# vfrantc/Bayesian-Enhancement-Model

Hardware: AMD Instinct MI355X
Metric: images/sec (whole node) CG_UNet N=8 Bayesian eval @256x256 (higher is better)
Workload: dtype f32

## Files before the change

bayesian-enhancement-model_amd/csrc/chan_attn.hip:

```cpp
#include "bem_common.h"

namespace {

constexpr int ATT_C = 32;
constexpr int ATT_CHUNK = 2048;
__global__ __launch_bounds__(256) void attn_stats_kernel(const float* __restrict__ f1, const float* __restrict__ f2,
                                                         double* __restrict__ stats, int L) {
    __shared__ double t1[ATT_C][65], t2[ATT_C][65];
    const int b = blockIdx.y;
    const int p0 = blockIdx.x * ATT_CHUNK;
    const int i0 = (threadIdx.x >> 4) * 2, j0 = (threadIdx.x & 15) * 2;
    double a00 = 0, a01 = 0, a10 = 0, a11 = 0, r0 = 0, r1 = 0, c0 = 0, c1 = 0;
    const float* F1 = f1 + (int64_t)b * ATT_C * L;
    const float* F2 = f2 + (int64_t)b * ATT_C * L;
    const int pend = min(p0 + ATT_CHUNK, L);
    for (int ps = p0; ps < pend; ps += 64) {
        __syncthreads();
        for (int i = threadIdx.x; i < ATT_C * 64; i += 256) {
            const int c = i >> 6, pp = i & 63;
            const int p = ps + pp;
            t1[c][pp] = p < pend ? (double)F1[(int64_t)c * L + p] : 0.0;
            t2[c][pp] = p < pend ? (double)F2[(int64_t)c * L + p] : 0.0;
        }
        __syncthreads();
#pragma unroll 8
        for (int pp = 0; pp < 64; ++pp) {
            const double u0 = t1[i0][pp], u1 = t1[i0 + 1][pp], v0 = t2[j0][pp], v1 = t2[j0 + 1][pp];
            a00 = fma(u0, v0, a00); a01 = fma(u0, v1, a01); a10 = fma(u1, v0, a10); a11 = fma(u1, v1, a11);
            if (j0 == 0) { r0 += u0; r1 += u1; }
            if (i0 == 0) { c0 += v0; c1 += v1; }
        }
    }
    double* S = stats + (int64_t)b * (ATT_C * ATT_C + 2 * ATT_C);
    atomicAdd(&S[i0 * ATT_C + j0], a00);
    atomicAdd(&S[i0 * ATT_C + j0 + 1], a01);
    atomicAdd(&S[(i0 + 1) * ATT_C + j0], a10);
    atomicAdd(&S[(i0 + 1) * ATT_C + j0 + 1], a11);
    if (j0 == 0) { atomicAdd(&S[ATT_C * ATT_C + i0], r0); atomicAdd(&S[ATT_C * ATT_C + i0 + 1], r1); }
    if (i0 == 0) { atomicAdd(&S[ATT_C * ATT_C + ATT_C + j0], c0); atomicAdd(&S[ATT_C * ATT_C + ATT_C + j0 + 1], c1); }
}

__device__ __forceinline__ double mm(const double (*A)[33], const double (*Bm)[33], int i, int j) {
    double s = 0;
#pragma unroll 8
    for (int k = 0; k < ATT_C; ++k) s = fma(A[i][k], Bm[k][j], s);
    return s;
}

__global__ __launch_bounds__(1024) void attn_fold_kernel(const double* __restrict__ stats, const float* __restrict__ aw,
                                                         const float* __restrict__ fw, const float* __restrict__ fb,
                                                         float* __restrict__ Wp, float* __restrict__ bias_out, int L) {
    __shared__ double X[ATT_C][33], Y[ATT_C][33], Z[ATT_C][33], M1[ATT_C][33], M2[ATT_C][33];
    __shared__ double va[ATT_C], vb[ATT_C], c1[ATT_C], c2[ATT_C], rowred[ATT_C];
    const int i = threadIdx.x >> 5, j = threadIdx.x & 31;
    const int b = blockIdx.x;
    const double* S = stats + (int64_t)b * (ATT_C * ATT_C + 2 * ATT_C);
    const double* s1 = S + ATT_C * ATT_C;
    const double* s2 = s1 + ATT_C;
    constexpr int WSZ = ATT_C * ATT_C + ATT_C;
    auto Wm = [&](int m, int r, int c) -> double { return (double)aw[m * WSZ + r * ATT_C + c]; };
    auto Bv = [&](int m, int r) -> double { return (double)aw[m * WSZ + ATT_C * ATT_C + r]; };
    const double scale = 1.0 / sqrt((double)ATT_C);
    for (int br = 0; br < 2; ++br) {
        const int mq = br ? 3 : 0, mk = br ? 4 : 1, mv = br ? 5 : 2, mo = br ? 7 : 6;
        const double* sq = br ? s2 : s1;
        const double* sk = br ? s1 : s2;
        __syncthreads();
        X[i][j] = br ? S[j * ATT_C + i] : S[i * ATT_C + j];
        Y[i][j] = Wm(mk, j, i);
        Z[i][j] = Wm(mq, i, j);
        if (i == 0) {
            double u = 0, t = 0;
            for (int k = 0; k < ATT_C; ++k) { u += Wm(mq, j, k) * sq[k]; t += Wm(mk, j, k) * sk[k]; }
            va[j] = u;
            vb[j] = t;
        }
        __syncthreads();
        const double t1 = mm(Z, X, i, j);
        __syncthreads();
        Z[i][j] = t1;
        __syncthreads();
        double g = mm(Z, Y, i, j);
        g += va[i] * Bv(mk, j) + Bv(mq, i) * vb[j] + (double)L * Bv(mq, i) * Bv(mk, j);
        g *= scale;
        __syncthreads();
        X[i][j] = g;
        __syncthreads();
        if (j == 0) {
            double m = X[i][0];
            for (int k = 1; k < ATT_C; ++k) m = fmax(m, X[i][k]);
            rowred[i] = m;
        }
        __syncthreads();
        const double e = exp(g - rowred[i]);
        __syncthreads();
        X[i][j] = e;
        __syncthreads();
        if (j == 0) {
            double s = 0;
            for (int k = 0; k < ATT_C; ++k) s += X[i][k];
            rowred[i] = s;
        }
        __syncthreads();
        const double pr = e / rowred[i];
        __syncthreads();
        X[i][j] = pr;
        Y[i][j] = Wm(mv, i, j);
        Z[i][j] = Wm(mo, i, j);
        __syncthreads();
        const double pv = mm(X, Y, i, j);
        if (j == 0) {
            double s = 0;
            for (int k = 0; k < ATT_C; ++k) s += X[i][k] * Bv(mv, k);
            va[i] = s;
        }
        __syncthreads();
        Y[i][j] = pv;
        __syncthreads();
        const double mres = mm(Z, Y, i, j);
        if (j == 0) {
            double s = Bv(mo, i);
            for (int k = 0; k < ATT_C; ++k) s += Z[i][k] * va[k];
            (br ? c2 : c1)[i] = s;
        }
        (br ? M2 : M1)[i][j] = mres;
    }
    __syncthreads();
    X[i][j] = (double)fw[i * 64 + j];
    Y[i][j] = (double)fw[i * 64 + 32 + j];
    __syncthreads();
    const double left = X[i][j] + mm(Y, M2, i, j);
    const double right = mm(X, M1, i, j) + Y[i][j];
    float* wp = Wp + (int64_t)b * (32 * 64);
    wp[i * 64 + j] = (float)left;
    wp[i * 64 + 32 + j] = (float)right;
    if (j == 0) {
        double s = (double)fb[i];
        for (int k = 0; k < ATT_C; ++k) s += X[i][k] * c1[k] + Y[i][k] * c2[k];
        bias_out[(int64_t)b * 32 + i] = (float)s;
    }
}

}

extern "C" int bem_attn_stats_f64(const float* f1, const float* f2, double* stats, int B, int L, void* stream) {
    BEM_REQUIRE(f1 && f2 && stats, "attn_stats: null tensor");
    BEM_REQUIRE(B >= 0 && B <= 65535 && L > 0, "attn_stats: bad shape");
    if (B == 0) return BEM_OK;
    hipStream_t s = (hipStream_t)stream;
    BEM_ZERO(stats, sizeof(double) * (size_t)B * (ATT_C * ATT_C + 2 * ATT_C), s, "attn_stats");
    dim3 grid(cdiv(L, ATT_CHUNK), B);
    attn_stats_kernel<<<grid, 256, 0, s>>>(f1, f2, stats, L);
    return bem_check_launch("attn_stats");
}

extern "C" int bem_attn_fold_f32(const double* stats, const float* attn_w, const float* fuse_w, const float* fuse_b,
                                 float* Wp_out, float* bias_out, int B, int L, void* stream) {
    BEM_REQUIRE(stats && attn_w && fuse_w && fuse_b && Wp_out && bias_out, "attn_fold: null tensor");
    BEM_REQUIRE(B >= 0 && L > 0, "attn_fold: bad shape");
    if (B == 0) return BEM_OK;
    attn_fold_kernel<<<B, 1024, 0, (hipStream_t)stream>>>(stats, attn_w, fuse_w, fuse_b, Wp_out, bias_out, L);
    return bem_check_launch("attn_fold");
}
```

bayesian-enhancement-model_amd/csrc/pack.hip:

```cpp
#include "bem_common.h"
#include "x6_common.h"

namespace {

__global__ void pack_pw_weight_kernel(const float* __restrict__ W, float* __restrict__ Wp, int M, int K, int MT, int KS) {
    const int64_t per = (int64_t)MT * KS * 64;
    const int64_t i = (int64_t)blockIdx.x * blockDim.x + threadIdx.x;
    if (i >= per) return;
    const int lane = (int)(i & 63);
    const int64_t t = i >> 6;
    const int st = (int)(t % KS), mt = (int)(t / KS);
    const int row = mt * 32 + (lane & 31), col = 2 * st + (lane >> 5);
    const int set = blockIdx.y;
    Wp[(int64_t)set * per + i] = (row < M && col < K) ? W[((int64_t)set * M + row) * K + col] : 0.f;
}

__device__ __forceinline__ void pack_x6_item(int64_t i, const float* __restrict__ W, u32x4* __restrict__ Wp, int M, int K, int MT, int KB,
                                             int64_t ss, int64_t rs, int64_t cs) {
    const int lane = (int)(i & 63);
    const int64_t blk = i >> 6;
    const int kb = (int)(blk % KB), mt = (int)((blk / KB) % MT);
    const int64_t set = blk / ((int64_t)KB * MT);
    const int row = mt * 32 + (lane & 31), k0 = kb * 16 + (lane >> 5) * 8;
    float v[8];
#pragma unroll
    for (int e = 0; e < 8; ++e) v[e] = (row < M && k0 + e < K) ? W[set * ss + row * rs + (k0 + e) * cs] : 0.f;
    u32x4 h, m, l;
    split8(v, h, m, l);
    u32x4* o = Wp + ((set * MT + mt) * KB + kb) * 3 * 64 + lane;
    o[0] = h; o[64] = m; o[128] = l;
}

__global__ void pack_x6_kernel(const float* __restrict__ W, u32x4* __restrict__ Wp, int M, int K, int MT, int KB, int64_t total,
                               int64_t ss, int64_t rs, int64_t cs) {
    const int64_t i = bem_gid1d();
    if (i >= total) return;
    pack_x6_item(i, W, Wp, M, K, MT, KB, ss, rs, cs);
}

struct packjob { const float* src; int64_t out; int32_t M, K; int64_t rs, cs, items, pad0, pad1; };
static_assert(sizeof(packjob) == 8 * 8, "packjob is eight 64-bit words (bem.modules.BayesBank builds it as an int64 table)");

__global__ __launch_bounds__(256) void pack_x6_jobs_kernel(const packjob* __restrict__ jobs, const int32_t* __restrict__ blks, float* __restrict__ arena) {
    const packjob jb = jobs[blks[2 * blockIdx.x]];
    const int64_t i = (int64_t)blks[2 * blockIdx.x + 1] * 256 + threadIdx.x;
    if (i >= jb.items) return;
    pack_x6_item(i, jb.src, reinterpret_cast<u32x4*>(arena + jb.out), jb.M, jb.K, (jb.M + 31) / 32, (jb.K + 15) / 16, 0, jb.rs, jb.cs);
}

__device__ __forceinline__ void sample_pack_x6_item(int64_t i, const float* __restrict__ mu, const float* __restrict__ rho,
                                                    const float* __restrict__ eps_in, u32x4* __restrict__ Wp, int M, int K, int MT, int KB,
                                                    uint64_t seed, uint64_t stream_id, int sigma_given) {
    const int lane = (int)(i & 63);
    const int64_t blk = i >> 6;
    const int kb = (int)(blk % KB), mt = (int)((blk / KB) % MT);
    const int64_t set = blk / ((int64_t)KB * MT);
    const int row = mt * 32 + (lane & 31), k0 = kb * 16 + (lane >> 5) * 8;
    float v[8];
    const int64_t g0 = set * M * K + (int64_t)row * K + k0;
    float z[3][4];
    if (!eps_in && row < M) {
#pragma unroll
        for (int q = 0; q < 3; ++q) philox_normal4((g0 >> 2) + q, seed, stream_id, z[q]);
    }
#pragma unroll
    for (int e = 0; e < 8; ++e) {
        v[e] = 0.f;
        if (row < M && k0 + e < K) {
            const int64_t idx = (int64_t)row * K + k0 + e, gi = g0 + e;
            const int off = (int)(g0 & 3);
            const float zsel = off == 0 ? z[e >> 2][e & 3] : off == 1 ? z[(e + 1) >> 2][(e + 1) & 3]
                             : off == 2 ? z[(e + 2) >> 2][(e + 2) & 3] : z[(e + 3) >> 2][(e + 3) & 3];
            const float eps = eps_in ? eps_in[gi] : zsel;
            v[e] = mu[idx] + (sigma_given ? rho[idx] : log1pf(expf(rho[idx]))) * eps;
        }
    }
    u32x4 h, m, l;
    split8(v, h, m, l);
    u32x4* o = Wp + ((set * MT + mt) * KB + kb) * 3 * 64 + lane;
    o[0] = h; o[64] = m; o[128] = l;
}

__global__ void sample_pack_x6_kernel(const float* __restrict__ mu, const float* __restrict__ rho, const float* __restrict__ eps_in,
                                      u32x4* __restrict__ Wp, int M, int K, int MT, int KB, int64_t total, uint64_t seed, uint64_t stream_id,
                                      const uint64_t* __restrict__ stream_add, int sigma_given) {
    const int64_t i = bem_gid1d();
    if (i >= total) return;
    if (stream_add) stream_id += stream_add[0];
    sample_pack_x6_item(i, mu, rho, eps_in, Wp, M, K, MT, KB, seed, stream_id, sigma_given);
}

__global__ void randn_kernel(float* __restrict__ out, int64_t total, uint64_t seed, uint64_t stream_id, const uint64_t* __restrict__ stream_add) {
    const int64_t i = bem_gid1d();
    if (stream_add) stream_id += stream_add[0];
    if (i < total) out[i] = philox_normal(i, seed, stream_id);
}

__global__ void bnn_sample_kernel(const float* __restrict__ mu, const float* __restrict__ rho,
                                  const float* __restrict__ eps_in, float* __restrict__ out, int64_t n, int64_t total,
                                  uint64_t seed, uint64_t stream_id, const uint64_t* __restrict__ stream_add) {
    const int64_t j = bem_gid1d();
    const int64_t i0 = 4 * j;
    if (i0 >= total) return;
    if (stream_add) stream_id += stream_add[0];
    float z[4] = {0.f, 0.f, 0.f, 0.f};
    if (!eps_in) philox_normal4(j, seed, stream_id, z);
#pragma unroll
    for (int q = 0; q < 4; ++q) {
        const int64_t i = i0 + q;
        if (i < total) {
            const int64_t e = i % n;
            const float eps = eps_in ? eps_in[i] : z[q];
            out[i] = mu[e] + log1pf(expf(rho[e])) * eps;
        }
    }
}

struct ebank_seg { const float* mu; const float* sig; int64_t out; int64_t n; int32_t M, K; uint64_t counter; int64_t items; int64_t total; };
static_assert(sizeof(ebank_seg) == 8 * 8, "ebank_seg is eight 64-bit words (bem.modules.EvalSampleBank builds it as an int64 table)");
struct ebank_blk { int32_t seg; int32_t first; };

__global__ __launch_bounds__(256) void ebank_sample_kernel(const ebank_seg* __restrict__ segs, const ebank_blk* __restrict__ blks,
                                                           float* __restrict__ arena, uint64_t seed, uint64_t stream_base) {
    const ebank_blk bk = blks[blockIdx.x];
    const ebank_seg sg = segs[bk.seg];
    const int64_t i = (int64_t)bk.first * 256 + threadIdx.x;
    if (i >= sg.items) return;
    const uint64_t sid = stream_base + sg.counter;
    float* out = arena + sg.out;
    if (sg.K > 0) {
        sample_pack_x6_item(i, sg.mu, sg.sig, nullptr, reinterpret_cast<u32x4*>(out), sg.M, sg.K, (sg.M + 31) / 32, (sg.K + 15) / 16, seed, sid, 1);
        return;
    }
    const int64_t i0 = 4 * i, total = sg.total;
    float z[4];
    philox_normal4(i, seed, sid, z);
#pragma unroll
    for (int q = 0; q < 4; ++q) {
        const int64_t e = i0 + q;
        if (e < total) {
            const int64_t k = e % sg.n;
            out[e] = sg.mu[k] + log1pf(expf(sg.sig[k])) * z[q];
        }
    }
}

}

extern "C" int64_t bem_pw_packed_elems(int M, int K) { return (int64_t)cdiv(M, 32) * cdiv(K, 2) * 64; }

extern "C" int bem_pack_pw_weight_f32(const float* W, float* Wp, int nsets, int M, int K, void* stream) {
    BEM_REQUIRE(W && Wp, "pack_pw_weight: null tensor");
    BEM_REQUIRE(nsets >= 0 && nsets <= 65535 && M > 0 && K > 0, "pack_pw_weight: bad shape");
    if (nsets == 0) return BEM_OK;
    const int MT = cdiv(M, 32), KS = cdiv(K, 2);
    dim3 grid((unsigned)cdiv64((int64_t)MT * KS * 64, 256), nsets);
    pack_pw_weight_kernel<<<grid, 256, 0, (hipStream_t)stream>>>(W, Wp, M, K, MT, KS);
    return bem_check_launch("pack_pw_weight");
}

extern "C" int bem_bnn_sample_f32(const float* mu, const float* rho, const float* eps_in, float* out, int nsets,
                                  int64_t n, uint64_t seed, uint64_t stream_id, const uint64_t* stream_add, void* stream) {
    BEM_REQUIRE(mu && rho && out, "bnn_sample: null tensor");
    BEM_REQUIRE(nsets >= 0 && n >= 0, "bnn_sample: bad shape");
    const int64_t total = (int64_t)nsets * n;
    if (total == 0) return BEM_OK;
    bnn_sample_kernel<<<GRID1D(cdiv64(total, 4)), 256, 0, (hipStream_t)stream>>>(mu, rho, eps_in, out, n, total, seed, stream_id, stream_add);
    return bem_check_launch("bnn_sample");
}

extern "C" int bem_randn_f32(float* out, int64_t n, uint64_t seed, uint64_t stream_id, const uint64_t* stream_add, void* stream) {
    BEM_REQUIRE(out && n >= 0, "randn: bad arguments");
    if (n == 0) return BEM_OK;
    randn_kernel<<<GRID1D(n), 256, 0, (hipStream_t)stream>>>(out, n, seed, stream_id, stream_add);
    return bem_check_launch("randn");
}

extern "C" int bem_bnn_ebank_sample_f32(const void* segs, const void* blks, int nblk, float* arena, uint64_t seed, uint64_t stream_base,
                                        void* stream) {
    BEM_REQUIRE(segs && blks && arena && nblk > 0, "bnn_ebank_sample: bad arguments");
    BEM_REQUIRE(((uintptr_t)arena & 15) == 0, "bnn_ebank_sample: the arena must be 16-byte aligned");
    ebank_sample_kernel<<<nblk, 256, 0, (hipStream_t)stream>>>((const ebank_seg*)segs, (const ebank_blk*)blks, arena, seed, stream_base);
    return bem_check_launch("bnn_ebank_sample");
}

extern "C" int bem_bnn_sample_pack_x6(const float* mu, const float* rho, const float* eps_in, float* Wp, int nsets, int M, int K,
                                      uint64_t seed, uint64_t stream_id, const uint64_t* stream_add, int sigma_given, void* stream) {
    BEM_REQUIRE(mu && rho && Wp, "bnn_sample_pack_x6: null tensor");
    BEM_REQUIRE(nsets >= 0 && M > 0 && K > 0, "bnn_sample_pack_x6: bad shape");
    BEM_REQUIRE(((uintptr_t)Wp & 15) == 0, "bnn_sample_pack_x6: output must be 16-byte aligned");
    if (nsets == 0) return BEM_OK;
    const int MT = cdiv(M, 32), KB = cdiv(K, 16);
    const int64_t total = (int64_t)nsets * MT * KB * 64;
    sample_pack_x6_kernel<<<GRID1D(total), 256, 0, (hipStream_t)stream>>>(mu, rho, eps_in, reinterpret_cast<u32x4*>(Wp), M, K, MT, KB,
                                                                                       total, seed, stream_id, stream_add, sigma_given);
    return bem_check_launch("bnn_sample_pack_x6");
}

extern "C" int64_t bem_pw_x6_packed_elems(int M, int K) {
    return (int64_t)cdiv(M, 32) * cdiv(K, 16) * 3 * 64 * 4;
}

extern "C" int bem_pack_pw_weight_x6_strided(const float* W, float* Wp, int nsets, int M, int K, int64_t set_stride, int64_t row_stride,
                                             int64_t col_stride, void* stream) {
    BEM_REQUIRE(W && Wp, "pack_pw_weight_x6: null tensor");
    BEM_REQUIRE(nsets >= 0 && M > 0 && K > 0 && set_stride >= 0 && row_stride >= 0 && col_stride >= 0, "pack_pw_weight_x6: bad shape / strides");
    BEM_REQUIRE(((uintptr_t)Wp & 15) == 0, "pack_pw_weight_x6: output must be 16-byte aligned");
    if (nsets == 0) return BEM_OK;
    const int MT = cdiv(M, 32), KB = cdiv(K, 16);
    const int64_t total = (int64_t)nsets * MT * KB * 64;
    pack_x6_kernel<<<GRID1D(total), 256, 0, (hipStream_t)stream>>>(W, reinterpret_cast<u32x4*>(Wp), M, K, MT, KB, total, set_stride,
                                                                                 row_stride, col_stride);
    return bem_check_launch("pack_pw_weight_x6");
}

extern "C" int bem_pack_pw_weight_x6_jobs(const void* jobs, const void* blks, int nblk, float* arena, void* stream) {
    BEM_REQUIRE(jobs && blks && arena && nblk > 0, "pack_pw_weight_x6_jobs: bad arguments");
    BEM_REQUIRE(((uintptr_t)arena & 15) == 0, "pack_pw_weight_x6_jobs: the arena must be 16-byte aligned");
    pack_x6_jobs_kernel<<<nblk, 256, 0, (hipStream_t)stream>>>((const packjob*)jobs, (const int32_t*)blks, arena);
    return bem_check_launch("pack_pw_weight_x6_jobs");
}

extern "C" int bem_pack_pw_weight_x6(const float* W, float* Wp, int nsets, int M, int K, void* stream) {
    return bem_pack_pw_weight_x6_strided(W, Wp, nsets, M, K, (int64_t)M * K, K, 1, stream);
}
```

Measured before the change: 357.9.

## Use f64 MFMA for channel-attention stats and streamline Bayesian weight sampling

Rewrites the channel-attention statistics kernel to compute the 32x32 cross-Gram matrix with f64 MFMA instructions. Each wave streams float4 loads directly from global memory with register double-buffering, and per-wave partials are reduced in shared memory before the atomics. Chunk size now shrinks adaptively so enough workgroups are launched for small batches. The sample-and-pack kernel gets an aligned fast path that skips unneeded Philox draws, uses vectorized mu/rho loads, and makes the block index wave-uniform via readfirstlane. Risks include MFMA summation-order differences in f64 and heavier register use.

```diff
diff --git a/bayesian-enhancement-model_amd/csrc/chan_attn.hip b/bayesian-enhancement-model_amd/csrc/chan_attn.hip
--- a/bayesian-enhancement-model_amd/csrc/chan_attn.hip
+++ b/bayesian-enhancement-model_amd/csrc/chan_attn.hip
@@ -3,41 +3,69 @@
 namespace {
 
 constexpr int ATT_C = 32;
-constexpr int ATT_CHUNK = 2048;
+constexpr int ATT_STATS = ATT_C * ATT_C + 2 * ATT_C;
+constexpr int ATT_CHUNK_MAX = 2048, ATT_CHUNK_MIN = 256;
+constexpr int ATT_MIN_WG = 512;
+using f64x4 = __attribute__((ext_vector_type(4))) double;
+
+__device__ __forceinline__ void att_load4(const float* __restrict__ row, int64_t p, int64_t pend, bool vec, float (&v)[4]) {
+    if (vec) {
+        const float4 t = p < pend ? *reinterpret_cast<const float4*>(row + p) : make_float4(0.f, 0.f, 0.f, 0.f);
+        v[0] = t.x; v[1] = t.y; v[2] = t.z; v[3] = t.w;
+    } else {
+#pragma unroll
+        for (int s = 0; s < 4; ++s) v[s] = p + s < pend ? row[p + s] : 0.f;
+    }
+}
+
 __global__ __launch_bounds__(256) void attn_stats_kernel(const float* __restrict__ f1, const float* __restrict__ f2,
-                                                         double* __restrict__ stats, int L) {
-    __shared__ double t1[ATT_C][65], t2[ATT_C][65];
-    const int b = blockIdx.y;
-    const int p0 = blockIdx.x * ATT_CHUNK;
-    const int i0 = (threadIdx.x >> 4) * 2, j0 = (threadIdx.x & 15) * 2;
-    double a00 = 0, a01 = 0, a10 = 0, a11 = 0, r0 = 0, r1 = 0, c0 = 0, c1 = 0;
-    const float* F1 = f1 + (int64_t)b * ATT_C * L;
-    const float* F2 = f2 + (int64_t)b * ATT_C * L;
-    const int pend = min(p0 + ATT_CHUNK, L);
-    for (int ps = p0; ps < pend; ps += 64) {
-        __syncthreads();
-        for (int i = threadIdx.x; i < ATT_C * 64; i += 256) {
-            const int c = i >> 6, pp = i & 63;
-            const int p = ps + pp;
-            t1[c][pp] = p < pend ? (double)F1[(int64_t)c * L + p] : 0.0;
-            t2[c][pp] = p < pend ? (double)F2[(int64_t)c * L + p] : 0.0;
+                                                         double* __restrict__ stats, int L, int chunk, int vec) {
+    __shared__ double part[4][ATT_STATS];
+    const int b = blockIdx.y, wave = threadIdx.x >> 6, lane = threadIdx.x & 63;
+    const int c = lane & 15, g = lane >> 4;
+    const int64_t p0 = (int64_t)blockIdx.x * chunk, pend = min(p0 + chunk, (int64_t)L);
+    const float* rows[4] = {f1 + ((int64_t)b * ATT_C + c) * L, f1 + ((int64_t)b * ATT_C + c + 16) * L,
+                            f2 + ((int64_t)b * ATT_C + c) * L, f2 + ((int64_t)b * ATT_C + c + 16) * L};
+    f64x4 acc[2][2] = {};
+    double sum[4] = {0, 0, 0, 0};
+    float cur[4][4], nxt[4][4];
+    int64_t pb = p0 + wave * 16;
+#pragma unroll
+    for (int r = 0; r < 4; ++r) att_load4(rows[r], pb + 4 * g, pend, vec, cur[r]);
+    for (; pb < pend; pb += 64) {
+#pragma unroll
+        for (int r = 0; r < 4; ++r) att_load4(rows[r], pb + 64 + 4 * g, pend, vec, nxt[r]);
+#pragma unroll
+        for (int s = 0; s < 4; ++s) {
+            const double a0 = (double)cur[0][s], a1 = (double)cur[1][s], b0 = (double)cur[2][s], b1 = (double)cur[3][s];
+            acc[0][0] = __builtin_amdgcn_mfma_f64_16x16x4f64(a0, b0, acc[0][0], 0, 0, 0);
+            acc[0][1] = __builtin_amdgcn_mfma_f64_16x16x4f64(a0, b1, acc[0][1], 0, 0, 0);
+            acc[1][0] = __builtin_amdgcn_mfma_f64_16x16x4f64(a1, b0, acc[1][0], 0, 0, 0);
+            acc[1][1] = __builtin_amdgcn_mfma_f64_16x16x4f64(a1, b1, acc[1][1], 0, 0, 0);
+            sum[0] += a0; sum[1] += a1; sum[2] += b0; sum[3] += b1;
         }
-        __syncthreads();
-#pragma unroll 8
-        for (int pp = 0; pp < 64; ++pp) {
-            const double u0 = t1[i0][pp], u1 = t1[i0 + 1][pp], v0 = t2[j0][pp], v1 = t2[j0 + 1][pp];
-            a00 = fma(u0, v0, a00); a01 = fma(u0, v1, a01); a10 = fma(u1, v0, a10); a11 = fma(u1, v1, a11);
-            if (j0 == 0) { r0 += u0; r1 += u1; }
-            if (i0 == 0) { c0 += v0; c1 += v1; }
-        }
+#pragma unroll
+        for (int r = 0; r < 4; ++r)
+#pragma unroll
+            for (int s = 0; s < 4; ++s) cur[r][s] = nxt[r][s];
     }
-    double* S = stats + (int64_t)b * (ATT_C * ATT_C + 2 * ATT_C);
-    atomicAdd(&S[i0 * ATT_C + j0], a00);
-    atomicAdd(&S[i0 * ATT_C + j0 + 1], a01);
-    atomicAdd(&S[(i0 + 1) * ATT_C + j0], a10);
-    atomicAdd(&S[(i0 + 1) * ATT_C + j0 + 1], a11);
-    if (j0 == 0) { atomicAdd(&S[ATT_C * ATT_C + i0], r0); atomicAdd(&S[ATT_C * ATT_C + i0 + 1], r1); }
-    if (i0 == 0) { atomicAdd(&S[ATT_C * ATT_C + ATT_C + j0], c0); atomicAdd(&S[ATT_C * ATT_C + ATT_C + j0 + 1], c1); }
+    double* mine = part[wave];
+#pragma unroll
+    for (int ti = 0; ti < 2; ++ti)
+#pragma unroll
+        for (int tj = 0; tj < 2; ++tj)
+#pragma unroll
+            for (int q = 0; q < 4; ++q) mine[(16 * ti + g + 4 * q) * ATT_C + 16 * tj + c] = acc[ti][tj][q];
+#pragma unroll
+    for (int r = 0; r < 4; ++r) {
+        double v = sum[r];
+        v += __shfl_xor(v, 16);
+        v += __shfl_xor(v, 32);
+        if (g == 0) mine[ATT_C * ATT_C + 16 * r + c] = v;
+    }
+    __syncthreads();
+    double* S = stats + (int64_t)b * ATT_STATS;
+    for (int i = threadIdx.x; i < ATT_STATS; i += 256) atomicAdd(&S[i], (part[0][i] + part[1][i]) + (part[2][i] + part[3][i]));
 }
 
 __device__ __forceinline__ double mm(const double (*A)[33], const double (*Bm)[33], int i, int j) {
@@ -148,9 +176,12 @@
     BEM_REQUIRE(B >= 0 && B <= 65535 && L > 0, "attn_stats: bad shape");
     if (B == 0) return BEM_OK;
     hipStream_t s = (hipStream_t)stream;
-    BEM_ZERO(stats, sizeof(double) * (size_t)B * (ATT_C * ATT_C + 2 * ATT_C), s, "attn_stats");
-    dim3 grid(cdiv(L, ATT_CHUNK), B);
-    attn_stats_kernel<<<grid, 256, 0, s>>>(f1, f2, stats, L);
+    BEM_ZERO(stats, sizeof(double) * (size_t)B * ATT_STATS, s, "attn_stats");
+    int chunk = ATT_CHUNK_MAX;
+    while (chunk > ATT_CHUNK_MIN && (int64_t)B * cdiv64(L, chunk) < ATT_MIN_WG) chunk >>= 1;
+    const int vec = L % 4 == 0 && (((uintptr_t)f1 | (uintptr_t)f2) & 15) == 0;
+    dim3 grid((unsigned)cdiv64(L, chunk), B);
+    attn_stats_kernel<<<grid, 256, 0, s>>>(f1, f2, stats, L, chunk, vec);
     return bem_check_launch("attn_stats");
 }
 
diff --git a/bayesian-enhancement-model_amd/csrc/pack.hip b/bayesian-enhancement-model_amd/csrc/pack.hip
--- a/bayesian-enhancement-model_amd/csrc/pack.hip
+++ b/bayesian-enhancement-model_amd/csrc/pack.hip
@@ -48,37 +48,62 @@
     pack_x6_item(i, jb.src, reinterpret_cast<u32x4*>(arena + jb.out), jb.M, jb.K, (jb.M + 31) / 32, (jb.K + 15) / 16, 0, jb.rs, jb.cs);
 }
 
+template <bool ALIGNED>
+__device__ __forceinline__ void sample_pack_x6_draw(int64_t set, int mt, int kb, int lane, const float* __restrict__ mu, const float* __restrict__ rho,
+                                                    const float* __restrict__ eps_in, u32x4* __restrict__ Wp, int M, int K, int MT, int KB,
+                                                    uint64_t seed, uint64_t stream_id, int sigma_given) {
+    const int row = mt * 32 + (lane & 31), k0 = kb * 16 + (lane >> 5) * 8;
+    float v[8];
+    const int64_t g0 = set * M * K + (int64_t)row * K + k0;
+    const int off = ALIGNED ? 0 : (int)(g0 & 3);
+    const int live = row < M ? min(8, K - k0) : 0;
+    constexpr int NQ = ALIGNED ? 2 : 3;
+    float z[NQ][4];
+#pragma unroll
+    for (int q = 0; q < NQ; ++q)
+        if (!eps_in && live > 0 && q <= ((off + live - 1) >> 2)) philox_normal4((g0 >> 2) + q, seed, stream_id, z[q]);
+    const int64_t idx0 = (int64_t)row * K + k0;
+    float mv[8], sv[8];
+    if (ALIGNED && (((uintptr_t)mu | (uintptr_t)rho) & 15) == 0) {
+#pragma unroll
+        for (int q = 0; q < 2; ++q) {
+            float4 a = make_float4(0.f, 0.f, 0.f, 0.f), b = a;
+            if (4 * q < live) { a = *reinterpret_cast<const float4*>(mu + idx0 + 4 * q); b = *reinterpret_cast<const float4*>(rho + idx0 + 4 * q); }
+            mv[4 * q] = a.x; mv[4 * q + 1] = a.y; mv[4 * q + 2] = a.z; mv[4 * q + 3] = a.w;
+            sv[4 * q] = b.x; sv[4 * q + 1] = b.y; sv[4 * q + 2] = b.z; sv[4 * q + 3] = b.w;
+        }
+    } else {
+#pragma unroll
+        for (int e = 0; e < 8; ++e) { mv[e] = e < live ? mu[idx0 + e] : 0.f; sv[e] = e < live ? rho[idx0 + e] : 0.f; }
+    }
+#pragma unroll
+    for (int e = 0; e < 8; ++e) {
+        v[e] = 0.f;
+        if (e < live) {
+            float zsel;
+            if constexpr (ALIGNED) zsel = z[e >> 2][e & 3];
+            else zsel = off == 0 ? z[e >> 2][e & 3] : off == 1 ? z[(e + 1) >> 2][(e + 1) & 3]
+                      : off == 2 ? z[(e + 2) >> 2][(e + 2) & 3] : z[(e + 3) >> 2][(e + 3) & 3];
+            const float eps = eps_in ? eps_in[g0 + e] : zsel;
+            v[e] = mv[e] + (sigma_given ? sv[e] : log1pf(expf(sv[e]))) * eps;
+        }
+    }
+    u32x4 h, m, l;
+    split8(v, h, m, l);
+    u32x4* o = Wp + ((set * MT + mt) * KB + kb) * 3 * 64 + lane;
+    o[0] = h; o[64] = m; o[128] = l;
+}
+
 __device__ __forceinline__ void sample_pack_x6_item(int64_t i, const float* __restrict__ mu, const float* __restrict__ rho,
                                                     const float* __restrict__ eps_in, u32x4* __restrict__ Wp, int M, int K, int MT, int KB,
                                                     uint64_t seed, uint64_t stream_id, int sigma_given) {
     const int lane = (int)(i & 63);
-    const int64_t blk = i >> 6;
+    const uint64_t ub = (uint64_t)(i >> 6);
+    const int64_t blk = (int64_t)(((uint64_t)__builtin_amdgcn_readfirstlane((uint32_t)(ub >> 32)) << 32) | __builtin_amdgcn_readfirstlane((uint32_t)ub));
     const int kb = (int)(blk % KB), mt = (int)((blk / KB) % MT);
     const int64_t set = blk / ((int64_t)KB * MT);
-    const int row = mt * 32 + (lane & 31), k0 = kb * 16 + (lane >> 5) * 8;
-    float v[8];
-    const int64_t g0 = set * M * K + (int64_t)row * K + k0;
-    float z[3][4];
-    if (!eps_in && row < M) {
-#pragma unroll
-        for (int q = 0; q < 3; ++q) philox_normal4((g0 >> 2) + q, seed, stream_id, z[q]);
-    }
-#pragma unroll
-    for (int e = 0; e < 8; ++e) {
-        v[e] = 0.f;
-        if (row < M && k0 + e < K) {
-            const int64_t idx = (int64_t)row * K + k0 + e, gi = g0 + e;
-            const int off = (int)(g0 & 3);
-            const float zsel = off == 0 ? z[e >> 2][e & 3] : off == 1 ? z[(e + 1) >> 2][(e + 1) & 3]
-                             : off == 2 ? z[(e + 2) >> 2][(e + 2) & 3] : z[(e + 3) >> 2][(e + 3) & 3];
-            const float eps = eps_in ? eps_in[gi] : zsel;
-            v[e] = mu[idx] + (sigma_given ? rho[idx] : log1pf(expf(rho[idx]))) * eps;
-        }
-    }
-    u32x4 h, m, l;
-    split8(v, h, m, l);
-    u32x4* o = Wp + ((set * MT + mt) * KB + kb) * 3 * 64 + lane;
-    o[0] = h; o[64] = m; o[128] = l;
+    if ((K & 3) == 0) sample_pack_x6_draw<true>(set, mt, kb, lane, mu, rho, eps_in, Wp, M, K, MT, KB, seed, stream_id, sigma_given);
+    else sample_pack_x6_draw<false>(set, mt, kb, lane, mu, rho, eps_in, Wp, M, K, MT, KB, seed, stream_id, sigma_given);
 }
 
 __global__ void sample_pack_x6_kernel(const float* __restrict__ mu, const float* __restrict__ rho, const float* __restrict__ eps_in,
```

Measured after the change: 363.1 (median of 6 runs). 1.01x the previous value.
